# WHDY/SceneDepthEstimation

Hardware: AMD Instinct MI355X
Metric: Mpixel-disparities/sec (H*W*D cost voxels per second, end-to-end per pair) (higher is better)
Workload: dtype f32; 1 GPU; north_star; H=1024, W=1024, D=192, C=64, nlayers=5, pipeline=tower+cv_wta, global_batch=1, parallelism=pairdp1

## Files before the change

include/sde.h:

```cpp
#ifndef SDE_H
#define SDE_H

#include <stddef.h>
#include <stdint.h>

#ifdef __cplusplus
extern "C" {
#endif

#define SDE_ABI_VERSION 4

typedef enum {
    SDE_OK = 0,
    SDE_ERR_ARG = -1,
    SDE_ERR_LAUNCH = -2,
    SDE_ERR_WORKSPACE = -3,
} sde_status;

typedef enum {
    SDE_LAYOUT_DHW = 0,
    SDE_LAYOUT_HWD = 1,
} sde_layout;

typedef enum {
// ... 35 lines not shown
int sde_argmin_merge(const float *mins, const int32_t *args, int nshards, int64_t npix, float *disp,
                     void *stream);


int sde_set_persistent_grid(int cus);

#define SDE_TOWER_FP32 0
#define SDE_TOWER_BF16X6 1
#define SDE_TOWER_F16X3 8
#define SDE_TOWER_WINOGRAD 16
#define SDE_TOWER_MFMA32 32
#define SDE_TOWER_IN_CBLOCK 2
#define SDE_TOWER_OUT_CBLOCK 4
#define SDE_TOWER_IN_SPLIT 64
#define SDE_TOWER_OUT_SPLIT 128

int64_t sde_tower_packed_floats(int nlayers, int nf);

int sde_tower_split_act(void);

int sde_tower_pack_weights(const float *const *hwio, const float *const *biases, int nlayers, int nf,
                           float *packed);

int64_t sde_tower_workspace_bytes(int H, int W, int nlayers, int nf);

int sde_tower_forward(const float *img_pad, int H, int W, const float *packed, int nlayers, int nf,
                      float *feat, void *workspace, int64_t workspace_bytes, int flags, uint16_t *feat_hi,
                      uint16_t *feat_lo, float *feat_norm, void *stream);

int64_t sde_tower_batch_workspace_bytes(int H, int W, int nimg, int nlayers, int nf);
// ... 10 lines not shown

int sde_tower_layer_batch(const float *in, int nimg, int64_t in_stride, int Hin, int Win, const float *packed,
                          int nlayers, int nf, int layer, float *out, int64_t out_stride, int flags,
                          const float *in_absmax, float *out_absmax, int amax_stride, void *stream);

int sde_absmax_f32_batch(const float *x, int nimg, int64_t n, float *absmax, int absmax_stride, void *stream);

int sde_absmax_f32(const float *x, int64_t n, float *absmax, void *stream);

int64_t sde_preprocess_scratch_bytes(int H, int W);
int sde_preprocess_u8(const uint8_t *img, int H, int W, int pad, float *out_pad, void *scratch,
                      void *stream);

int sde_preprocess_u8_batch(const uint8_t *imgs, int nimg, int H, int W, int pad, float *out_pad, void *scratch,
                            void *stream);


int sde_sgm_penalties(const uint8_t *img, int H, int W, double P1, double P2, int64_t threshold,
                      double lambda, float *pen, void *stream);

int sde_sgm_8path(const float *cv, const float *pen, int H, int W, int D, float *S, void *stream);

#define SDE_SGM_ACCUMULATE 1
#define SDE_SGM_ZERO_DU_PENALTIES 2
int sde_sgm_8path_pair(const float *cv_l, const float *pen_l, float *S_l, const float *cv_r, const float *pen_r,
                       float *S_r, int H, int W, int D, int flags, void *stream);

int sde_sgm_8path_wta_pair(const float *cv_l, const float *pen_l, float *S_l, float *disp_l, const float *cv_r,
                           const float *pen_r, float *S_r, float *disp_r, int H, int W, int D, int flags,
                           void *stream);
// ... 36 lines not shown
```

scenedepthestimation_amd/_lib.py:

```python
from __future__ import annotations

import ctypes
import os
import re

import torch

from ._build import INCLUDE, LIB

c_int, c_int64, c_float, c_double, c_void_p = ctypes.c_int, ctypes.c_int64, ctypes.c_float, ctypes.c_double, ctypes.c_void_p
c_char_p = ctypes.c_char_p

SDE_OK = 0
SDE_ABI_VERSION = 4
SDE_LAYOUT_DHW, SDE_LAYOUT_HWD = 0, 1
SDE_WTA_INIT_INF, SDE_WTA_INIT_D0 = 0, 1
SDE_SIDE_LEFT, SDE_SIDE_RIGHT = 1, 2
SDE_TOWER_FP32, SDE_TOWER_BF16X6, SDE_TOWER_F16X3 = 0, 1, 8
SDE_TOWER_IN_CBLOCK, SDE_TOWER_OUT_CBLOCK = 2, 4
SDE_TOWER_WINOGRAD = 16
SDE_TOWER_MFMA32 = 32
SDE_TOWER_IN_SPLIT, SDE_TOWER_OUT_SPLIT = 64, 128
SDE_CV_EXACT, SDE_CV_CERTIFIED = 0, 1
SDE_SGM_ACCUMULATE = 1
SDE_SGM_ZERO_DU_PENALTIES = 2

SIGNATURES = {
    "sde_abi_version": (c_int, []),
    "sde_status_string": (c_char_p, [c_int]),
    "sde_cost_volume": (c_int, [c_void_p, c_void_p, c_int, c_int, c_int, c_int, c_int, c_int, c_float,
                                c_void_p, c_void_p, c_void_p]),
    "sde_wta": (c_int, [c_void_p, c_int, c_int, c_int, c_int, c_int, c_void_p, c_void_p]),
    "sde_cv_wta_workspace_bytes": (c_int64, [c_int, c_int]),
    "sde_cv_wta": (c_int, [c_void_p, c_void_p, c_int, c_int, c_int, c_int, c_int, c_void_p, c_void_p,
                           c_void_p, c_int, c_void_p, c_int64, c_void_p]),
    "sde_feature_split": (c_int, [c_void_p, c_int64, c_int, c_void_p, c_void_p, c_void_p, c_void_p]),
    "sde_cv_wta_split_workspace_bytes": (c_int64, [c_int, c_int]),
# ... 8 lines not shown
    "sde_tower_forward": (c_int, [c_void_p, c_int, c_int, c_void_p, c_int, c_int, c_void_p, c_void_p,
                                  c_int64, c_int, c_void_p, c_void_p, c_void_p, c_void_p]),
    "sde_tower_layer": (c_int, [c_void_p, c_int, c_int, c_void_p, c_int, c_int, c_int, c_void_p, c_int, c_void_p,
                                c_void_p, c_void_p, c_void_p]),
    "sde_tower_batch_workspace_bytes": (c_int64, [c_int, c_int, c_int, c_int, c_int]),
    "sde_tower_forward_batch": (c_int, [c_void_p, c_int, c_int, c_int, c_void_p, c_int, c_int, c_void_p, c_void_p,
                                        c_int64, c_int, c_void_p, c_void_p, c_void_p, c_void_p]),
    "sde_tower_layer_scaled": (c_int, [c_void_p, c_int, c_int, c_void_p, c_int, c_int, c_int, c_void_p, c_int,
                                       c_void_p, c_void_p, c_void_p, c_void_p, c_void_p, c_void_p]),
    "sde_tower_layer_batch": (c_int, [c_void_p, c_int, c_int64, c_int, c_int, c_void_p, c_int, c_int, c_int,
                                      c_void_p, c_int64, c_int, c_void_p, c_void_p, c_int, c_void_p]),
    "sde_absmax_f32": (c_int, [c_void_p, c_int64, c_void_p, c_void_p]),
    "sde_set_persistent_grid": (c_int, [c_int]),
    "sde_absmax_f32_batch": (c_int, [c_void_p, c_int, c_int64, c_void_p, c_int, c_void_p]),
    "sde_preprocess_u8_batch": (c_int, [c_void_p, c_int, c_int, c_int, c_int, c_void_p, c_void_p, c_void_p]),
    "sde_preprocess_u8": (c_int, [c_void_p, c_int, c_int, c_int, c_void_p, c_void_p, c_void_p]),
    "sde_preprocess_scratch_bytes": (c_int64, [c_int, c_int]),
    "sde_sgm_penalties": (c_int, [c_void_p, c_int, c_int, c_double, c_double, c_int64, c_double, c_void_p,
                                  c_void_p]),
    "sde_sgm_8path": (c_int, [c_void_p, c_void_p, c_int, c_int, c_int, c_void_p, c_void_p]),
    "sde_sgm_8path_pair": (c_int, [c_void_p] * 6 + [c_int, c_int, c_int, c_int, c_void_p]),
    "sde_sgm_8path_wta_pair": (c_int, [c_void_p] * 8 + [c_int, c_int, c_int, c_int, c_void_p]),
    "sde_sgm_direction": (c_int, [c_void_p, c_void_p, c_int, c_int, c_int, c_int, c_void_p, c_void_p]),
    "sde_cbca_arms": (c_int, [c_void_p, c_int64, c_int, c_int, c_int, ctypes.c_float, c_void_p, c_void_p]),
    "sde_cbca_workspace_bytes": (ctypes.c_size_t, [c_int, c_int]),
    "sde_cbca": (c_int, [c_void_p] * 4 + [c_int] * 6 + [c_void_p, ctypes.c_size_t, c_void_p]),
    "sde_cbca_pair": (c_int, [c_void_p] * 6 + [c_int] * 5 + [c_void_p, ctypes.c_size_t, c_void_p]),
    "sde_cbca_lr": (c_int, [c_void_p] * 5 + [c_int] * 5 + [c_void_p, ctypes.c_size_t, c_void_p]),
    "sde_cbca_reciprocals": (c_int, [c_void_p, c_int, c_void_p]),
    "sde_lr_check": (c_int, [c_void_p, c_void_p, c_int, c_int, c_void_p, c_void_p, c_void_p]),
# ... 45 lines not shown
```

scenedepthestimation_amd/csrc/cost_volume.hip:

```cpp
#include "sde_common.h"
#include "cv_cert.h"

#include <algorithm>

namespace sde {

constexpr int CV_TX = 64;
constexpr int CV_WAVES = 4;
constexpr int CV_DC = 64;
constexpr int CV_DW = CV_DC / CV_WAVES;
constexpr int CV_ROWS = CV_TX + CV_DC - 1;

enum { OUT_WTA = 0, OUT_DHW = 1, OUT_HWD = 2 };

constexpr int CV_RSTRIDE = 17;

__device__ __forceinline__ float dot64_exact(const float (&own)[64], const float4 *__restrict__ win, int lr)
{
    float acc[8];
    const float4 *row = win + lr * CV_RSTRIDE;
#pragma unroll
    for (int m = 0; m < 8; m++) {
        const float4 a = row[2 * m];
        const float4 b = row[2 * m + 1];
// ... 811 lines not shown
    if (H <= 0 || W <= 0 || d0 < 0 || d1 <= d0 || (!disp && !min_cost && !argmin)) return SDE_ERR_ARG;
    if (!workspace || workspace_bytes < cert_ws_bytes(H, W, false)) return SDE_ERR_WORKSPACE;
    hipStream_t st = as_stream(stream);
    unsigned *counter = reinterpret_cast<unsigned *>(workspace);
    int32_t *list = reinterpret_cast<int32_t *>(reinterpret_cast<char *>(workspace) + 256);
    if (hipMemsetAsync(counter, 0, CERT_COUNTERS * sizeof(unsigned), st) != hipSuccess) return SDE_ERR_LAUNCH;
    cv_wta_cert_kernel<<<cdiv(W, FX_NX) * H, 256, 0, st>>>(
        fl, fr, reinterpret_cast<const uint4 *>(fl_hi), reinterpret_cast<const uint4 *>(fl_lo), fl_norm,
        reinterpret_cast<const uint4 *>(fr_hi), reinterpret_cast<const uint4 *>(fr_lo), fr_norm, H, W, d0, d1,
        min_cost, argmin, disp, counter, list);
    cv_wta_fixup_kernel<<<1024, 256, 0, st>>>(fl, fr, W, d0, d1, counter, list, min_cost, argmin, disp);
    return launch_status();
}

constexpr int ROW_CHUNK = 256;

SDE_EXPORT int sde_cv_wta(const float *fl, const float *fr, int H, int W, int C, int d0, int d1, float *disp,
                          float *min_cost, int32_t *argmin, int mode, void *workspace, int64_t workspace_bytes,
                          void *stream)
{
    if (!fl || !fr || H <= 0 || W <= 0 || C <= 0 || d0 < 0 || d1 <= d0) return SDE_ERR_ARG;
    if (!disp && !min_cost && !argmin) return SDE_ERR_ARG;
    if (mode != SDE_CV_EXACT && mode != SDE_CV_CERTIFIED) return SDE_ERR_ARG;
    hipStream_t st = as_stream(stream);
    auto exact64 = [&] {
        dim3 grid(cdiv(W, CV_TX), H);
        cv64_kernel<SDE_SIDE_LEFT, OUT_WTA><<<grid, 256, 0, st>>>(fl, fr, H, W, d0, d1, 0, -0.0f, nullptr, min_cost,
                                                                   argmin, disp);
    };
    if (C == 64 && mode == SDE_CV_CERTIFIED) {
        if (!workspace || workspace_bytes < sde_cv_wta_workspace_bytes(H, W)) return SDE_ERR_WORKSPACE;
        const int64_t npix = (int64_t)H * W;
        const int K = cdiv(d1 - d0, ROW_CHUNK);
        unsigned *counter = reinterpret_cast<unsigned *>(workspace);
        int32_t *list = reinterpret_cast<int32_t *>(reinterpret_cast<char *>(workspace) + 256);
        if (hipMemsetAsync(counter, 0, CERT_COUNTERS * sizeof(unsigned), st) != hipSuccess) return SDE_ERR_LAUNCH;
        if (row_cert_supported(d0, d1)) {
            launch_row_cert(fl, fr, H, W, d0, d1, min_cost, argmin, disp, counter, list, st);
            cv_wta_fixup_kernel<<<1024, 256, 0, st>>>(fl, fr, W, d0, d1, counter, list, min_cost, argmin, disp);
        } else if (K <= CERT_COUNTERS) {
            float *cmin = reinterpret_cast<float *>(reinterpret_cast<char *>(workspace) + cert_ws_bytes(H, W, false));
            int32_t *carg = reinterpret_cast<int32_t *>(cmin + (size_t)K * npix);
            for (int k = 0; k < K; k++) {
                const int a = d0 + k * ROW_CHUNK, b = std::min(d1, a + ROW_CHUNK);
                float *mk = cmin + (size_t)k * npix;
                int32_t *ak = carg + (size_t)k * npix;
                launch_row_cert(fl, fr, H, W, a, b, mk, ak, nullptr, counter + k, list, st, k > 0 ? mk - npix : nullptr);
                cv_wta_fixup_kernel<<<1024, 256, 0, st>>>(fl, fr, W, a, b, counter + k, list, mk, ak, nullptr);
            }
            argmin_chunks_kernel<<<cdiv(npix, 256), 256, 0, st>>>(cmin, carg, K, npix, disp, min_cost, argmin);
        } else {
            exact64();
        }
    } else if (C == 64) {
        exact64();
// ... 37 lines not shown
```

scenedepthestimation_amd/csrc/cv_row.hip:

```cpp
#include "cv_cert.h"

#include <algorithm>
#include <type_traits>

namespace sde {

constexpr int RW_S = 8;
constexpr float RW_SCALE = (float)(1 << RW_S);
constexpr float RW_K = 1.5e-5f;
constexpr float RW_ABS = 9.3132257e-10f;
constexpr float RW_NMAX = 127.0f;
typedef _Float16 rw_f16x8 __attribute__((ext_vector_type(8)));

__device__ __forceinline__ void rw_split(float x, _Float16 &h, _Float16 &l)
{
    const float xs = x * RW_SCALE;
    h = (_Float16)xs;
    l = (_Float16)(xs - (float)h);
}

__device__ __forceinline__ void rw_split2(float x0, float x1, uint32_t &hi, uint32_t &lo)
{
    typedef _Float16 h2 __attribute__((ext_vector_type(2)));
    const h2 hh = {(_Float16)x0, (_Float16)x1};
    hi = __builtin_bit_cast(uint32_t, hh);
    asm("v_fma_mixlo_f16 %0, %1, 1.0, -%2 op_sel_hi:[0,0,1]" : "=&v"(lo) : "v"(x0), "v"(hi));
    asm("v_fma_mixhi_f16 %0, %1, 1.0, -%2 op_sel:[0,0,1] op_sel_hi:[0,0,1]" : "+v"(lo) : "v"(x1), "v"(hi));
}

constexpr int RW_T = 32;

__device__ __forceinline__ float4 rw_load(const float *__restrict__ frrow, int W, int T, int u)
{
    const int xr = T * RW_T + (u >> 4);
    const bool ok = xr >= 0 && xr < W;
    const float4 v = reinterpret_cast<const float4 *>(frrow)[(size_t)(ok ? xr : 0) * 16 + (u & 15)];
    return ok ? v : make_float4(0.f, 0.f, 0.f, 0.f);
}

template <int CTRL>
__device__ __forceinline__ float rw_dpp(float v)
{
    return __int_as_float(__builtin_amdgcn_update_dpp(0, __float_as_int(v), CTRL, 0xF, 0xF, false));
}

__device__ __forceinline__ bool rw_nonfinite(float x) { return (__float_as_uint(x) & 0x7f800000u) == 0x7f800000u; }

constexpr int R2_NX = 128;
constexpr int R2_NEW = R2_NX / RW_T;
constexpr int R2_LEAD = 2;

__device__ __forceinline__ void r2_load(const float *__restrict__ frrow, int W, int T, int lane, float4 (&v)[8])
{
#pragma unroll
    for (int i = 0; i < 8; i++) v[i] = rw_load(frrow, W, T, lane + 64 * i);
}

__device__ __forceinline__ void r2_store(uint4 *ring, unsigned *tmax, unsigned *tbad, int slot, int lane,
                                         const float4 (&v)[8])
{
    unsigned mx = 0u;
    bool bad = false;
#pragma unroll
    for (int i = 0; i < 8; i++) {
        const int u = lane + 64 * i, px = u >> 4, q = u & 15;
        char *base = reinterpret_cast<char *>(ring + slot * 512 + fx_slot(px, q >> 1)) + 8 * (q & 1);
        const float xs[4] = {v[i].x * RW_SCALE, v[i].y * RW_SCALE, v[i].z * RW_SCALE, v[i].w * RW_SCALE};
        uint32_t hw[2], lw[2];
#pragma unroll
        for (int e = 0; e < 2; e++) rw_split2(xs[2 * e], xs[2 * e + 1], hw[e], lw[e]);
// ... 22 lines not shown
                                                          float *__restrict__ out_min, int32_t *__restrict__ out_arg,
                                                          float *__restrict__ out_disp, unsigned *__restrict__ counter,
                                                          int32_t *__restrict__ list, const float *__restrict__ prev_min)
{
    extern __shared__ __attribute__((aligned(16))) uint4 rsm2[];
    uint4 *ring = rsm2;
    unsigned *tmax = reinterpret_cast<unsigned *>(ring + nt * 512);
    unsigned *tbad = tmax + nt;
    const int y = blockIdx.x;
    const int tid = threadIdx.x, lane = tid & 63;
    const int wave = __builtin_amdgcn_readfirstlane(tid >> 6);
    const int j = lane & 31, h = lane >> 5;
    const float *flrow = fl + (size_t)y * W * 64;
    const float *frrow = fr + (size_t)y * W * 64;
    const size_t rowpix = (size_t)y * W;
    const int nss = (W + R2_NX - 1) / R2_NX;
    auto slot_of = [&](int T) { int r = T % nt; return r < 0 ? r + nt : r; };

    if (wave >= 4) {
        const int sw = wave - 4;
        constexpr int PB = 4;
        float4 nv[8];
#pragma unroll
        for (int b = 0; b < 4 / PB; b++) {
            float4 pv[PB][8];
#pragma unroll
            for (int i = 0; i < PB; i++)
                if (sw + 4 * (PB * b + i) < nw) r2_load(frrow, W, tlo0 + sw + 4 * (PB * b + i), lane, pv[i]);
            if (b == 4 / PB - 1 && nss > 1) r2_load(frrow, W, tlo0 + nw + sw, lane, nv);
#pragma unroll
            for (int i = 0; i < PB; i++)
                if (sw + 4 * (PB * b + i) < nw) r2_store(ring, tmax, tbad, slot_of(tlo0 + sw + 4 * (PB * b + i)), lane, pv[i]);
        }
        __syncthreads();
        for (int k = 0; k < nss; k++) {
            if (k + 1 < nss) {
                const int T = tlo0 + R2_NEW * (k + 1) + nw - R2_NEW + sw;
                r2_store(ring, tmax, tbad, slot_of(T), lane, nv);
                if (k + 2 < nss) r2_load(frrow, W, T + R2_NEW, lane, nv);
            }
            __syncthreads();
        }
        return;
    }

    const int grp = wave & 3;
    float4 lraw[8];
    auto load_left = [&](int kk) {
        const int xx = kk * R2_NX + RW_T * grp + j;
        const float4 *src = reinterpret_cast<const float4 *>(flrow) + (size_t)(xx < W ? xx : 0) * 16 + 2 * h;
#pragma unroll
        for (int s2 = 0; s2 < 4; s2++) { lraw[2 * s2] = src[4 * s2]; lraw[2 * s2 + 1] = src[4 * s2 + 1]; }
    };
    load_left(0);
// ... 243 lines not shown
```

scenedepthestimation_amd/csrc/preprocess.hip:

```cpp
#include "sde_common.h"
#include <algorithm>

namespace sde {

constexpr int NP_PIECE = 8192;

__device__ __forceinline__ float np_val(const uint8_t *img, int64_t i, float mean, bool sq)
{
    const float x = (float)img[i];
    if (!sq) return x;
    const float d = x - mean;
    return d * d;
}

__device__ float np_leaf(const uint8_t *img, int64_t s, int len, float mean, bool sq)
{
    if (len < 8) {
        float res = 0.0f;
        for (int i = 0; i < len; i++) res += np_val(img, s + i, mean, sq);
        return res;
    }
    float r[8];
#pragma unroll
    for (int j = 0; j < 8; j++) r[j] = np_val(img, s + j, mean, sq);
    int i = 8;
    for (; i < len - (len % 8); i += 8) {
#pragma unroll
        for (int j = 0; j < 8; j++) r[j] += np_val(img, s + i + j, mean, sq);
    }
    float res = ((r[0] + r[1]) + (r[2] + r[3])) + ((r[4] + r[5]) + (r[6] + r[7]));
    for (; i < len; i++) res += np_val(img, s + i, mean, sq);
    return res;
}

__device__ __forceinline__ int np_half(int len) { const int n2 = len / 2; return n2 - n2 % 8; }

__device__ __forceinline__ float np_stat(const float *__restrict__ v, int npieces, int64_t n, float *buf, int lane)
{
    float q = 0.0f;
    for (int c0 = 0; c0 < npieces; c0 += 256) {
        const int m = min(256, npieces - c0);
        for (int c = lane; c < m; c += 64) buf[c] = v[c0 + c];
        __builtin_amdgcn_wave_barrier();
        __builtin_amdgcn_fence(__ATOMIC_RELEASE, "wavefront");
        __builtin_amdgcn_wave_barrier();
        if (lane == 0)
            for (int c = 0; c < m; c++) q += buf[c];
        __builtin_amdgcn_wave_barrier();
        __builtin_amdgcn_fence(__ATOMIC_RELEASE, "wavefront");
        __builtin_amdgcn_wave_barrier();
    }
    q = __shfl(q, 0, 64);
    return (float)((double)q / (double)n);
}

template <bool SQ>
__global__ __launch_bounds__(64) void np_piece_kernel(const uint8_t *__restrict__ imgs, int64_t n, int sstride,
                                                      float *__restrict__ scratch)
{
    const uint8_t *img = imgs + blockIdx.y * n;
    float *st = scratch + (size_t)blockIdx.y * sstride;
    const int npieces = gridDim.x;
    __shared__ float sbuf[256];
    float mean = 0.0f;
    if (SQ) {
        mean = np_stat(st + 4, npieces, n, sbuf, threadIdx.x);
        if (blockIdx.x == 0 && threadIdx.x == 0) st[0] = mean;
    }
    const int lane = threadIdx.x;
    const int64_t c0 = (int64_t)blockIdx.x * NP_PIECE;
    const int m = (int)std::min<int64_t>(NP_PIECE, n - c0);
    float sum;
    if (m == NP_PIECE) {
        sum = np_leaf(img, c0 + 128 * lane, 128, mean, SQ);
#pragma unroll
        for (int o = 1; o < 64; o <<= 1) sum += __shfl_xor(sum, o, 64);
    } else {
        __shared__ float leaf[256];
        {
            int ss[16], sl[16], sp = 0, k = 0;
            ss[0] = 0; sl[0] = m;
            while (sp >= 0) {
                const int s0 = ss[sp], len = sl[sp];
                sp--;
                if (len <= 128) {
                    if ((k & 63) == lane) leaf[k] = np_leaf(img, c0 + s0, len, mean, SQ);
                    k++;
                } else {
                    const int n2 = np_half(len);
                    ss[++sp] = s0 + n2; sl[sp] = len - n2;
                    ss[++sp] = s0; sl[sp] = n2;
                }
            }
        }
        __syncthreads();
        sum = 0.0f;
        if (lane == 0) {
            int fl[16], fs[16], sp = 0, k = 0;
            float fv[16], ret = 0.0f;
            fl[0] = m; fs[0] = 0;
            while (sp >= 0) {
// ... 8 lines not shown
                } else if (fs[sp] == 1) {
                    fv[sp] = ret;
                    fs[sp] = 2;
                    const int n2 = np_half(len);
                    ++sp; fl[sp] = len - n2; fs[sp] = 0;
                    continue;
                } else {
                    ret = fv[sp] + ret;
                    sp--;
                }
            }
            sum = ret;
        }
    }
    if (lane == 0) st[4 + (SQ ? npieces : 0) + blockIdx.x] = sum;
}

constexpr int ZN_PER = 8;

__global__ __launch_bounds__(256) void znorm_pad_kernel(const uint8_t *__restrict__ img, int H, int W, int pad,
                                                        float *__restrict__ scratch, int sstride, int npieces,
                                                        float *__restrict__ out)
{
    const int Wp = W + 2 * pad;
    img += (size_t)blockIdx.y * H * W;
    float *st = scratch + (size_t)blockIdx.y * sstride;
    out += (size_t)blockIdx.y * (H + 2 * pad) * Wp;
    __shared__ float sbuf[256];
    __shared__ float sstd;
    if (threadIdx.x < 64) {
        const float v = sqrtf(np_stat(st + 4 + npieces, npieces, (int64_t)H * W, sbuf, threadIdx.x));
        if (threadIdx.x == 0) {
            sstd = v;
            if (blockIdx.x == 0) st[1] = v;
        }
    }
    __syncthreads();
    const float mean = st[0], stdv = sstd;
    const int64_t np_ = (int64_t)(H + 2 * pad) * Wp;
#pragma unroll
    for (int k = 0; k < ZN_PER; k++) {
        const int64_t i = ((int64_t)blockIdx.x * ZN_PER + k) * blockDim.x + threadIdx.x;
        if (i >= np_) break;
        const int ii = (int)i;
        const int y = ii / Wp - pad, x = ii % Wp - pad;
        float v = 0.0f;
        if (y >= 0 && y < H && x >= 0 && x < W) v = ((float)img[(size_t)y * W + x] - mean) / stdv;
        out[i] = v;
    }
}

}

using namespace sde;

SDE_EXPORT int64_t sde_preprocess_scratch_bytes(int H, int W)
{
    if (H <= 0 || W <= 0) return -1;
    const int64_t pieces = ((int64_t)H * W + NP_PIECE - 1) / NP_PIECE;
    return ((4 + 2 * pieces) * 4 + 255) / 256 * 256;
}

SDE_EXPORT int sde_preprocess_u8_batch(const uint8_t *imgs, int nimg, int H, int W, int pad, float *out_pad,
                                       void *scratch, void *stream)
{
    if (!imgs || !out_pad || !scratch || nimg <= 0 || nimg > 65535 || H <= 0 || W <= 0 || pad < 0) return SDE_ERR_ARG;
    const int64_t n = (int64_t)(H + 2 * pad) * (W + 2 * pad);
    if (n >= ((int64_t)1 << 31)) return SDE_ERR_ARG;
    hipStream_t st = as_stream(stream);
    const int64_t npix = (int64_t)H * W;
    const int pieces = (int)((npix + NP_PIECE - 1) / NP_PIECE);
    const int sstride = (int)(sde_preprocess_scratch_bytes(H, W) / 4);
    float *sc = reinterpret_cast<float *>(scratch);
    np_piece_kernel<false><<<dim3(pieces, nimg), 64, 0, st>>>(imgs, npix, sstride, sc);
    np_piece_kernel<true><<<dim3(pieces, nimg), 64, 0, st>>>(imgs, npix, sstride, sc);
    znorm_pad_kernel<<<dim3((unsigned)cdiv(n, 256 * ZN_PER), nimg), 256, 0, st>>>(imgs, H, W, pad, sc, sstride, pieces,
                                                                                  out_pad);
    return launch_status();
}

SDE_EXPORT int sde_preprocess_u8(const uint8_t *img, int H, int W, int pad, float *out_pad, void *scratch,
                                 void *stream)
{
    return sde_preprocess_u8_batch(img, 1, H, W, pad, out_pad, scratch, stream);
}
```

scenedepthestimation_amd/csrc/tower.hip:

```cpp
#include "tower_launch.h"
#include <algorithm>
#include <atomic>

namespace sde {

__global__ __launch_bounds__(256) void absmax_kernel(const float *__restrict__ x, int64_t n, float *__restrict__ amax,
                                                     int amax_stride)
{
    x += blockIdx.y * n;
    amax += blockIdx.y * amax_stride;
    float m = 0.0f;
    const int64_t tid = (int64_t)blockIdx.x * blockDim.x + threadIdx.x, nt = (int64_t)gridDim.x * blockDim.x;
    const int64_t head = std::min<int64_t>(n, (16 - (reinterpret_cast<uintptr_t>(x) & 15)) / 4 & 3);
    if (tid < head) m = fabsf(x[tid]);
    const float4 *x4 = reinterpret_cast<const float4 *>(x + head);
    const int64_t n4 = (n - head) / 4;
    for (int64_t i = tid; i < n4; i += nt) {
        const float4 v = x4[i];
        m = fmaxf(m, fmaxf(fmaxf(fabsf(v.x), fabsf(v.y)), fmaxf(fabsf(v.z), fabsf(v.w))));
    }
    for (int64_t i = head + 4 * n4 + tid; i < n; i += nt) m = fmaxf(m, fabsf(x[i]));
#pragma unroll
    for (int o = 32; o > 0; o >>= 1) m = fmaxf(m, __shfl_xor(m, o, 64));
    __shared__ float red[4];
// ... 98 lines not shown
static bool split_ok(int nlayers, int64_t pix) { return nlayers <= XP_SCALE_WORD && pix < SPLIT_MAX_PIX; }
static bool split_pairing_ok(bool in_sp, bool out_sp, int layer, int nlayers, int Hin, int Win)
{
    if (!in_sp && !out_sp) return true;
    const int sh = layer == 2 ? 4 : 2;
    if ((in_sp && !split_ok(nlayers, (int64_t)Hin * Win)) || (out_sp && !split_ok(nlayers, (int64_t)(Hin - sh) * (Win - sh))))
        return false;
    if ((in_sp && layer == 2) || (out_sp && layer == nlayers)) return false;
    return layer == 2 || layer == nlayers || in_sp == out_sp;
}

SDE_EXPORT int sde_tower_split_act(void) { return SDE_SPLIT_ACT; }

static bool tower_flags_ok(int flags, bool layer_api)
{
    if (flags & (SDE_TOWER_IN_SPLIT | SDE_TOWER_OUT_SPLIT)) {
        if (!layer_api || !(flags & SDE_TOWER_F16X3) || (flags & (SDE_TOWER_WINOGRAD | SDE_TOWER_MFMA32))) return false;
        if ((flags & SDE_TOWER_IN_SPLIT && flags & SDE_TOWER_IN_CBLOCK) ||
            (flags & SDE_TOWER_OUT_SPLIT && flags & SDE_TOWER_OUT_CBLOCK)) return false;
        flags &= ~(SDE_TOWER_IN_SPLIT | SDE_TOWER_OUT_SPLIT);
    }
    if (flags & (SDE_TOWER_WINOGRAD | SDE_TOWER_MFMA32)) {
        if (!(flags & SDE_TOWER_F16X3) || (flags & SDE_TOWER_WINOGRAD && flags & SDE_TOWER_MFMA32)) return false;
        flags &= ~(SDE_TOWER_WINOGRAD | SDE_TOWER_MFMA32);
    }
    const int prec = flags & (SDE_TOWER_BF16X6 | SDE_TOWER_F16X3);
    if (prec == (SDE_TOWER_BF16X6 | SDE_TOWER_F16X3)) return false;
    const int layout = SDE_TOWER_IN_CBLOCK | SDE_TOWER_OUT_CBLOCK;
    if (!layer_api) return (flags & ~(SDE_TOWER_BF16X6 | SDE_TOWER_F16X3)) == 0;
    if (flags & ~(SDE_TOWER_BF16X6 | SDE_TOWER_F16X3 | layout)) return false;
// ... 97 lines not shown
        return launch_status();
    }
    float *buf[2] = {nullptr, nullptr};
    const int64_t h2 = H + 2 * (nlayers - 2), w2 = W + 2 * (nlayers - 2);
    const int64_t act_stride = h2 * w2 * NF;
    if (nlayers > 2) {
        buf[0] = reinterpret_cast<float *>(workspace);
        buf[1] = buf[0] + nimg * act_stride;
    }
    float *amax = reinterpret_cast<float *>(static_cast<char *>(workspace) +
                                            (nlayers > 2 ? 2 * nimg * act_stride * 4 : 0));
    constexpr int AS = (int)(TOWER_AMAX_BYTES / 4);
    const bool f16 = (flags & SDE_TOWER_F16X3) != 0;
    if (f16) {
        if (nlayers > AS) return SDE_ERR_ARG;
        if (hipMemsetAsync(amax, 0, nimg * TOWER_AMAX_BYTES, st) != hipSuccess) return SDE_ERR_LAUNCH;
        const int blocks = (int)std::min<int64_t>(std::max<int64_t>(1, 256 / nimg), cdiv(img_stride, 256 * 16));
        absmax_kernel<<<dim3(blocks, nimg), 256, 0, st>>>(img_pad, img_stride, amax, AS);
    }
    int hin = Hp, win = Wp;
    const bool sp = SDE_SPLIT_ACT && f16 && !(flags & (SDE_TOWER_WINOGRAD | SDE_TOWER_MFMA32)) && nlayers > 2 &&
                    split_ok(nlayers, h2 * w2);
    const bool cbl = !sp && (flags & (SDE_TOWER_BF16X6 | SDE_TOWER_F16X3)) != 0;
    TowerLaunch L{};
    L.ohi = feat_hi, L.olo = feat_lo, L.onrm = feat_norm, L.nimg = nimg, L.bt.amax_stride = AS, L.st = st;
    for (int l = 2; l <= nlayers; l++) {
        const bool first = l == 2, last = l == nlayers;
        L.in = first ? img_pad : buf[(l & 1) ^ 1], L.Hin = hin, L.Win = win, L.out = last ? feat : buf[l & 1];
        L.bt.in_stride = first ? img_stride : act_stride, L.bt.out_stride = last ? feat_stride : act_stride;
        L.in_amax = amax + (l - 2), L.out_amax = amax + (l - 1);
// ... 15 lines not shown
```

scenedepthestimation_amd/ops.py:

```python
from __future__ import annotations

import ctypes

import numpy as np
import torch

from . import _lib
from ._lib import (SDE_LAYOUT_DHW, SDE_LAYOUT_HWD, SDE_SIDE_LEFT, SDE_SIDE_RIGHT, SDE_WTA_INIT_D0,
                   SDE_WTA_INIT_INF, check, lib)

LAYOUTS = {"DHW": SDE_LAYOUT_DHW, "HWD": SDE_LAYOUT_HWD}
RULES = {"inf": SDE_WTA_INIT_INF, "d0": SDE_WTA_INIT_D0}


def _stream() -> int:
    return torch.cuda.current_stream().cuda_stream


def _need(t: torch.Tensor, name: str, dtype=torch.float32, shape=None):
    if not isinstance(t, torch.Tensor):
        raise TypeError(f"{name} must be a torch.Tensor")
    if not t.is_cuda:
        raise ValueError(f"{name} must live on the GPU (got {t.device}); libsde has no CPU path")
    if t.dtype != dtype:
# ... 215 lines not shown
def absmax(x, out):
    check(lib.sde_absmax_f32(_need(x, "absmax input"), x.numel(), _need(out, "absmax word", shape=(1,)), _stream()),
          "sde_absmax_f32")
    return out


def set_persistent_grid(cus: int = 0):
    check(lib.sde_set_persistent_grid(int(cus)), "sde_set_persistent_grid")


def tower_batch_workspace_bytes(H: int, W: int, nimg: int, nlayers: int, nf: int = 64) -> int:
    return int(lib.sde_tower_batch_workspace_bytes(H, W, nimg, nlayers, nf))


def tower_forward_batch(img_pad, packed, nlayers: int, nf: int = 64, out=None, workspace=None,
                        precision: str = "f16x3"):
    N, Hp, Wp = img_pad.shape
    H, W = Hp - 2 * nlayers, Wp - 2 * nlayers
    if H <= 0 or W <= 0:
        raise ValueError("padded image smaller than the tower's receptive field")
    pi = _need(img_pad, "img_pad")
    pw = _need(packed, "packed weights", shape=(tower_packed_floats(nlayers, nf),))
    if out is None:
        out = _empty((N, H, W, nf), torch.float32, img_pad)
    po = _need(out, "features", shape=(N, H, W, nf))
    need = tower_batch_workspace_bytes(H, W, N, nlayers, nf)
    if need > 0 and workspace is None:
        workspace = torch.empty(need, dtype=torch.uint8, device=img_pad.device)
    pws = _need(workspace, "workspace", dtype=torch.uint8) if need > 0 else None
    wsb = workspace.numel() if need > 0 else 0
    check(lib.sde_tower_forward_batch(pi, N, H, W, pw, nlayers, nf, po, pws, wsb, TOWER_PRECISIONS[precision],
                                      None, None, None, _stream()), "sde_tower_forward_batch")
    return out


def absmax_batch(x, out):
    N = x.shape[0]
    _need(x, "absmax input")
    if out.dtype != torch.float32 or not out.is_cuda or out.shape[0] != N or out.stride(1) != 1:
        raise ValueError("absmax words must be a float32 [N, k] device tensor with unit column stride")
    check(lib.sde_absmax_f32_batch(x.data_ptr(), N, x[0].numel(), out.data_ptr(), out.stride(0), _stream()),
          "sde_absmax_f32_batch")
    return out


SCALE_WORD = 32
AMAX_ROW_WORDS = 64
TOWER_SPLIT_ACT = bool(lib.sde_tower_split_act())
# ... 86 lines not shown

def preprocess_u8(img_u8, pad: int, out=None, stats=None):
    H, W = img_u8.shape
    pi = _need(img_u8, "image", dtype=torch.uint8)
    nb = preprocess_scratch_bytes(H, W)
    if out is None:
        out = _empty((H + 2 * pad, W + 2 * pad), torch.float32, img_u8)
    if stats is None:
        stats = _empty((nb,), torch.uint8, img_u8)
    check(lib.sde_preprocess_u8(pi, H, W, pad, _need(out, "out_pad", shape=(H + 2 * pad, W + 2 * pad)),
                                _need(stats, "scratch", dtype=torch.uint8, shape=(nb,)),
                                _stream()), "sde_preprocess_u8")
    return out


def preprocess_u8_batch(imgs_u8, pad: int, out=None, stats=None):
    N, H, W = imgs_u8.shape
    pi = _need(imgs_u8, "images", dtype=torch.uint8)
    nb = N * preprocess_scratch_bytes(H, W)
    if out is None:
        out = _empty((N, H + 2 * pad, W + 2 * pad), torch.float32, imgs_u8)
    if stats is None:
        stats = _empty((nb,), torch.uint8, imgs_u8)
    check(lib.sde_preprocess_u8_batch(pi, N, H, W, pad, _need(out, "out_pad", shape=(N, H + 2 * pad, W + 2 * pad)),
                                      _need(stats, "scratch", dtype=torch.uint8, shape=(nb,)),
                                      _stream()), "sde_preprocess_u8_batch")
    return out


def sgm_penalties(img_u8, P1=2.3, P2=55.9, threshold=30, lamda=4, out=None):
    H, W = img_u8.shape
    pi = _need(img_u8, "image", dtype=torch.uint8)
    if out is None:
        out = _empty((H, W, 16), torch.float32, img_u8)
    check(lib.sde_sgm_penalties(pi, H, W, float(P1), float(P2), int(threshold), float(lamda),
                                _need(out, "penalties", shape=(H, W, 16)), _stream()), "sde_sgm_penalties")
    return out


def sgm_8path(cv_hwd, pen, S=None):
    H, W, D = cv_hwd.shape
# ... 148 lines not shown
```

scenedepthestimation_amd/pipeline.py:

```python
from __future__ import annotations

import numpy as np
import torch

from . import mc_cnn, ops


AMAX_WORDS = ops.AMAX_ROW_WORDS
SPLIT_MAX_PIX = 1 << 24
SGM_PLACEMENT_TRIALS = 16
SGM_PLACEMENT_MIN_VOXELS = 1 << 26
SGM_PLACEMENT_MAX_VOXELS = 1 << 29


def tower_steps(img_pad, packed, nlayers: int, out, ws, precision: str = "f16x3", nf: int = 64, on_launch=None):
    L = nlayers
    N, Hp, Wp = img_pad.shape
    H, W = Hp - 2 * L, Wp - 2 * L
    need = ops.tower_batch_workspace_bytes(H, W, N, L, nf)
    if ws.numel() < need:
        raise ValueError("tower workspace too small")
    h2, w2 = H + 2 * (L - 2), W + 2 * (L - 2)
    sp = ops.TOWER_SPLIT_ACT and precision == "f16x3" and 2 < L <= ops.SCALE_WORD and h2 * w2 < SPLIT_MAX_PIX
    cbl = not sp and precision in ("bf16x6", "f16x3", "f16x3w", "f16x3m32")
    act = h2 * w2 * nf if L > 2 else 0
    wsf = ws[: 2 * N * act * 4 + N * AMAX_WORDS * 4].view(torch.float32)
    bufs = [wsf[: N * act], wsf[N * act: 2 * N * act]]
    words = wsf[2 * N * act:].view(N, AMAX_WORDS)
    f16 = precision in ("f16x3", "f16x3w", "f16x3m32")
    if f16:
        words.zero_()
        ops.absmax_batch(img_pad, words)
    yield 1, words

    def run(layer, fn):
        if on_launch is None:
            fn()
        else:
            on_launch(layer, fn)

    hin, win = H + 2 * L - 4, W + 2 * L - 4
    first = out if L == 2 else bufs[0][: N * hin * win * nf].view(N, hin, win, nf)
    run(2, lambda: ops.tower_layer_batch(img_pad, packed, L, 2, first, nf=nf, precision=precision,
                                         out_cblock=cbl and L > 2, in_absmax=words[:, 0:1] if f16 else None,
                                         out_absmax=words[:, 1:2] if (f16 and L > 2) else None, out_split=sp))
    cur = 0
    for layer in range(3, L + 1):
        yield layer - 1, words
        src = bufs[cur][: N * hin * win * nf].view(N, hin, win, nf)
        o = out if layer == L else bufs[cur ^ 1][: N * (hin - 2) * (win - 2) * nf].view(N, hin - 2, win - 2, nf)
        run(layer, lambda: ops.tower_layer_batch(src, packed, L, layer, o, nf=nf, precision=precision,
                                                 in_cblock=cbl, out_cblock=cbl and layer < L,
                                                 in_absmax=words[:, layer - 2:layer - 1] if f16 else None,
                                                 out_absmax=words[:, layer - 1:layer] if (f16 and layer < L) else None,
                                                 in_split=sp, out_split=sp and layer < L))
        hin, win = hin - 2, win - 2
        cur ^= 1


def run_tower(img_pad, packed, nlayers, out, ws, precision="f16x3", nf=64, combine=None, on_launch=None):
    for _stage, words in tower_steps(img_pad, packed, nlayers, out, ws, precision, nf, on_launch):
        if combine is not None:
            combine(words)
    return out


class StereoMatcher:
    def __init__(self, height: int, width: int, ndisp: int, weights=None, nlayers: int = 5,
                 nf: int = 64, device=None, d_range=None, sgm: bool = False, tower_precision: str = "f16x3",
                 cv_mode: str = "certified", cbca_iters: int = 0, cbca_L1: int = 14, cbca_tau: float = 0.02,
                 emit_split: bool = False, sgm_placement_trials: int = SGM_PLACEMENT_TRIALS):
        self.H, self.W, self.D = int(height), int(width), int(ndisp)
        self.cbca_iters, self.cbca_L1, self.cbca_tau = int(cbca_iters), int(cbca_L1), float(cbca_tau)
        self.nlayers, self.nf = int(nlayers), int(nf)
        self.sgm_placement_trials = int(sgm_placement_trials)
        self.sgm_placement_ms = None
# ... 31 lines not shown
            self._alloc_sgm()

    @property
    def ws(self):
        if self._ws is None:
            nws = ops.tower_batch_workspace_bytes(self.H, self.W, 2, self.nlayers, self.nf)
            self._ws = torch.empty(max(nws, 1), dtype=torch.uint8, device=self.device)
        return self._ws

    def load_images(self, left_u8, right_u8):
        for dst, src in zip(self.img_u8, (left_u8, right_u8)):
            t = src if isinstance(src, torch.Tensor) else torch.from_numpy(np.ascontiguousarray(src, np.uint8))
            dst.copy_(t, non_blocking=False)

    def features(self, on_launch=None):
        ops.preprocess_u8_batch(self.img_u82, self.nlayers, out=self.img_pad2, stats=self.stats2)
        return self.features_from_padded(on_launch)

    def features_from_padded(self, on_launch=None):
        if on_launch is not None and self.split:
            raise ValueError("on_launch needs the layer-by-layer tower, which does not emit split planes "
                             "(emit_split=True): time the one-call tower instead")
        if on_launch is not None:
            run_tower(self.img_pad2, self.packed, self.nlayers, self.feat2, self.ws, self.tower_precision, self.nf,
                      on_launch=on_launch)
            self.split_valid = False
            return self.feat[0], self.feat[1]
        if self.split:
            for i in range(2):
                ops.tower_forward(self.img_pad[i], self.packed, self.nlayers, self.nf, out=self.feat[i],
                                  workspace=self.ws, precision=self.tower_precision, split=self.split[i])
        else:
            ops.tower_forward_batch(self.img_pad2, self.packed, self.nlayers, self.nf, out=self.feat2,
                                    workspace=self.ws, precision=self.tower_precision)
        self.split_valid = self.split is not None
        return self.feat[0], self.feat[1]

    def cost_wta(self, want=("disp",)):
        if self.cv_mode == "certified" and self.split_valid:
            return ops.cv_wta_split(self.feat[0], self.feat[1], self.split[0], self.split[1], self.d0, self.d1,
                                    disp=self.disp if "disp" in want else None,
                                    min_cost=self.min_cost if "min" in want else None,
                                    argmin=self.argmin if "argmin" in want else None, want=(),
                                    workspace=self.cv_ws)
        return ops.cv_wta(self.feat[0], self.feat[1], self.d0, self.d1,
                          disp=self.disp if "disp" in want else None,
                          min_cost=self.min_cost if "min" in want else None,
                          argmin=self.argmin if "argmin" in want else None, want=(),
                          mode=self.cv_mode, workspace=self.cv_ws)
# ... 125 lines not shown
```

Before: 117,900 Mpixel-disparities/s.

## Fuse input absmax into preprocess and use buffer loads in row cost-volume kernel

Preprocessing now tracks the per-image min/max pixel and writes the normalized absmax bound into the tower's amax workspace, so the f16x3 tower can skip its own memset and absmax pass over the padded image. Separately, the row-certified cost-volume kernel swaps guarded global float4 loads for raw buffer loads with a hardware range check, which removes per-load bounds arithmetic. The buffer path is restricted to widths below a limit so the 32-bit offsets stay valid. The added min/max tracking and atomics in preprocessing are a small extra cost.

```diff
diff --git a/include/sde.h b/include/sde.h
--- a/include/sde.h
+++ b/include/sde.h
@@ -73,6 +73,7 @@
 #define SDE_TOWER_OUT_CBLOCK 4
 #define SDE_TOWER_IN_SPLIT 64
 #define SDE_TOWER_OUT_SPLIT 128
+#define SDE_TOWER_BOUND_READY 256
 
 int64_t sde_tower_packed_floats(int nlayers, int nf);
 
@@ -113,6 +114,9 @@
 
 int sde_preprocess_u8_batch(const uint8_t *imgs, int nimg, int H, int W, int pad, float *out_pad, void *scratch,
                             void *stream);
+
+int sde_preprocess_u8_bound_batch(const uint8_t *imgs, int nimg, int H, int W, int pad, float *out_pad, void *scratch,
+                                  float *amax, int amax_stride, int amax_words, void *stream);
 
 
 int sde_sgm_penalties(const uint8_t *img, int H, int W, double P1, double P2, int64_t threshold,
diff --git a/scenedepthestimation_amd/_lib.py b/scenedepthestimation_amd/_lib.py
--- a/scenedepthestimation_amd/_lib.py
+++ b/scenedepthestimation_amd/_lib.py
@@ -21,6 +21,7 @@
 SDE_TOWER_WINOGRAD = 16
 SDE_TOWER_MFMA32 = 32
 SDE_TOWER_IN_SPLIT, SDE_TOWER_OUT_SPLIT = 64, 128
+SDE_TOWER_BOUND_READY = 256
 SDE_CV_EXACT, SDE_CV_CERTIFIED = 0, 1
 SDE_SGM_ACCUMULATE = 1
 SDE_SGM_ZERO_DU_PENALTIES = 2
@@ -59,6 +60,8 @@
     "sde_set_persistent_grid": (c_int, [c_int]),
     "sde_absmax_f32_batch": (c_int, [c_void_p, c_int, c_int64, c_void_p, c_int, c_void_p]),
     "sde_preprocess_u8_batch": (c_int, [c_void_p, c_int, c_int, c_int, c_int, c_void_p, c_void_p, c_void_p]),
+    "sde_preprocess_u8_bound_batch": (c_int, [c_void_p, c_int, c_int, c_int, c_int, c_void_p, c_void_p, c_void_p,
+                                              c_int, c_int, c_void_p]),
     "sde_preprocess_u8": (c_int, [c_void_p, c_int, c_int, c_int, c_void_p, c_void_p, c_void_p]),
     "sde_preprocess_scratch_bytes": (c_int64, [c_int, c_int]),
     "sde_sgm_penalties": (c_int, [c_void_p, c_int, c_int, c_double, c_double, c_int64, c_double, c_void_p,
diff --git a/scenedepthestimation_amd/csrc/cost_volume.hip b/scenedepthestimation_amd/csrc/cost_volume.hip
--- a/scenedepthestimation_amd/csrc/cost_volume.hip
+++ b/scenedepthestimation_amd/csrc/cost_volume.hip
@@ -849,6 +849,7 @@
 }
 
 constexpr int ROW_CHUNK = 256;
+constexpr int ROW_MAX_W = 1 << 23;
 
 SDE_EXPORT int sde_cv_wta(const float *fl, const float *fr, int H, int W, int C, int d0, int d1, float *disp,
                           float *min_cost, int32_t *argmin, int mode, void *workspace, int64_t workspace_bytes,
@@ -870,10 +871,10 @@
         unsigned *counter = reinterpret_cast<unsigned *>(workspace);
         int32_t *list = reinterpret_cast<int32_t *>(reinterpret_cast<char *>(workspace) + 256);
         if (hipMemsetAsync(counter, 0, CERT_COUNTERS * sizeof(unsigned), st) != hipSuccess) return SDE_ERR_LAUNCH;
-        if (row_cert_supported(d0, d1)) {
+        if (W < ROW_MAX_W && row_cert_supported(d0, d1)) {
             launch_row_cert(fl, fr, H, W, d0, d1, min_cost, argmin, disp, counter, list, st);
             cv_wta_fixup_kernel<<<1024, 256, 0, st>>>(fl, fr, W, d0, d1, counter, list, min_cost, argmin, disp);
-        } else if (K <= CERT_COUNTERS) {
+        } else if (W < ROW_MAX_W && K <= CERT_COUNTERS) {
             float *cmin = reinterpret_cast<float *>(reinterpret_cast<char *>(workspace) + cert_ws_bytes(H, W, false));
             int32_t *carg = reinterpret_cast<int32_t *>(cmin + (size_t)K * npix);
             for (int k = 0; k < K; k++) {
diff --git a/scenedepthestimation_amd/csrc/cv_row.hip b/scenedepthestimation_amd/csrc/cv_row.hip
--- a/scenedepthestimation_amd/csrc/cv_row.hip
+++ b/scenedepthestimation_amd/csrc/cv_row.hip
@@ -30,12 +30,18 @@
 
 constexpr int RW_T = 32;
 
-__device__ __forceinline__ float4 rw_load(const float *__restrict__ frrow, int W, int T, int u)
-{
-    const int xr = T * RW_T + (u >> 4);
-    const bool ok = xr >= 0 && xr < W;
-    const float4 v = reinterpret_cast<const float4 *>(frrow)[(size_t)(ok ? xr : 0) * 16 + (u & 15)];
-    return ok ? v : make_float4(0.f, 0.f, 0.f, 0.f);
+__device__ __forceinline__ __amdgpu_buffer_rsrc_t rw_rsrc(const float *row, int W)
+{
+    const uintptr_t b = (uintptr_t)row;
+    const uint32_t lo = __builtin_amdgcn_readfirstlane((uint32_t)b);
+    const uint32_t hi = __builtin_amdgcn_readfirstlane((uint32_t)(b >> 32));
+    return __builtin_amdgcn_make_buffer_rsrc((void *)(((uintptr_t)hi << 32) | lo), 0,
+                                             (int)__builtin_amdgcn_readfirstlane((uint32_t)W * 256u), 0x00020000);
+}
+
+__device__ __forceinline__ float4 rw_load(__amdgpu_buffer_rsrc_t row, uint32_t off)
+{
+    return __builtin_bit_cast(float4, __builtin_amdgcn_raw_buffer_load_b128(row, off, 0, 0));
 }
 
 template <int CTRL>
@@ -50,10 +56,11 @@
 constexpr int R2_NEW = R2_NX / RW_T;
 constexpr int R2_LEAD = 2;
 
-__device__ __forceinline__ void r2_load(const float *__restrict__ frrow, int W, int T, int lane, float4 (&v)[8])
-{
-#pragma unroll
-    for (int i = 0; i < 8; i++) v[i] = rw_load(frrow, W, T, lane + 64 * i);
+__device__ __forceinline__ void r2_load(__amdgpu_buffer_rsrc_t frrow, int T, int lane, float4 (&v)[8])
+{
+    const uint32_t base = (uint32_t)T * (RW_T * 256u) + 16u * (uint32_t)lane;
+#pragma unroll
+    for (int i = 0; i < 8; i++) v[i] = rw_load(frrow, base + 1024u * i);
 }
 
 __device__ __forceinline__ void r2_store(uint4 *ring, unsigned *tmax, unsigned *tbad, int slot, int lane,
@@ -106,6 +113,7 @@
     const float *flrow = fl + (size_t)y * W * 64;
     const float *frrow = fr + (size_t)y * W * 64;
     const size_t rowpix = (size_t)y * W;
+    const __amdgpu_buffer_rsrc_t frbuf = rw_rsrc(frrow, W);
     const int nss = (W + R2_NX - 1) / R2_NX;
     auto slot_of = [&](int T) { int r = T % nt; return r < 0 ? r + nt : r; };
 
@@ -118,8 +126,8 @@
             float4 pv[PB][8];
 #pragma unroll
             for (int i = 0; i < PB; i++)
-                if (sw + 4 * (PB * b + i) < nw) r2_load(frrow, W, tlo0 + sw + 4 * (PB * b + i), lane, pv[i]);
-            if (b == 4 / PB - 1 && nss > 1) r2_load(frrow, W, tlo0 + nw + sw, lane, nv);
+                if (sw + 4 * (PB * b + i) < nw) r2_load(frbuf, tlo0 + sw + 4 * (PB * b + i), lane, pv[i]);
+            if (b == 4 / PB - 1 && nss > 1) r2_load(frbuf, tlo0 + nw + sw, lane, nv);
 #pragma unroll
             for (int i = 0; i < PB; i++)
                 if (sw + 4 * (PB * b + i) < nw) r2_store(ring, tmax, tbad, slot_of(tlo0 + sw + 4 * (PB * b + i)), lane, pv[i]);
@@ -129,7 +137,7 @@
             if (k + 1 < nss) {
                 const int T = tlo0 + R2_NEW * (k + 1) + nw - R2_NEW + sw;
                 r2_store(ring, tmax, tbad, slot_of(T), lane, nv);
-                if (k + 2 < nss) r2_load(frrow, W, T + R2_NEW, lane, nv);
+                if (k + 2 < nss) r2_load(frbuf, T + R2_NEW, lane, nv);
             }
             __syncthreads();
         }
diff --git a/scenedepthestimation_amd/csrc/preprocess.hip b/scenedepthestimation_amd/csrc/preprocess.hip
--- a/scenedepthestimation_amd/csrc/preprocess.hip
+++ b/scenedepthestimation_amd/csrc/preprocess.hip
@@ -5,31 +5,38 @@
 
 constexpr int NP_PIECE = 8192;
 
-__device__ __forceinline__ float np_val(const uint8_t *img, int64_t i, float mean, bool sq)
-{
-    const float x = (float)img[i];
+struct NpRange {
+    unsigned lo = 255u, hi = 0u;
+};
+
+__device__ __forceinline__ float np_val(const uint8_t *img, int64_t i, float mean, bool sq, NpRange &r)
+{
+    const unsigned px = img[i];
+    const float x = (float)px;
     if (!sq) return x;
+    r.lo = min(r.lo, px);
+    r.hi = max(r.hi, px);
     const float d = x - mean;
     return d * d;
 }
 
-__device__ float np_leaf(const uint8_t *img, int64_t s, int len, float mean, bool sq)
+__device__ float np_leaf(const uint8_t *img, int64_t s, int len, float mean, bool sq, NpRange &rg)
 {
     if (len < 8) {
         float res = 0.0f;
-        for (int i = 0; i < len; i++) res += np_val(img, s + i, mean, sq);
+        for (int i = 0; i < len; i++) res += np_val(img, s + i, mean, sq, rg);
         return res;
     }
     float r[8];
 #pragma unroll
-    for (int j = 0; j < 8; j++) r[j] = np_val(img, s + j, mean, sq);
+    for (int j = 0; j < 8; j++) r[j] = np_val(img, s + j, mean, sq, rg);
     int i = 8;
     for (; i < len - (len % 8); i += 8) {
 #pragma unroll
-        for (int j = 0; j < 8; j++) r[j] += np_val(img, s + i + j, mean, sq);
+        for (int j = 0; j < 8; j++) r[j] += np_val(img, s + i + j, mean, sq, rg);
     }
     float res = ((r[0] + r[1]) + (r[2] + r[3])) + ((r[4] + r[5]) + (r[6] + r[7]));
-    for (; i < len; i++) res += np_val(img, s + i, mean, sq);
+    for (; i < len; i++) res += np_val(img, s + i, mean, sq, rg);
     return res;
 }
 
@@ -56,11 +63,18 @@
 
 template <bool SQ>
 __global__ __launch_bounds__(64) void np_piece_kernel(const uint8_t *__restrict__ imgs, int64_t n, int sstride,
-                                                      float *__restrict__ scratch)
+                                                      float *__restrict__ scratch, float *__restrict__ amax,
+                                                      int amax_stride, int amax_words)
 {
     const uint8_t *img = imgs + blockIdx.y * n;
     float *st = scratch + (size_t)blockIdx.y * sstride;
+    unsigned *range = reinterpret_cast<unsigned *>(st + 2);
     const int npieces = gridDim.x;
+    if (!SQ && amax && blockIdx.x == 0) {
+        for (int w = threadIdx.x; w < amax_words; w += 64) amax[(size_t)blockIdx.y * amax_stride + w] = 0.0f;
+        if (threadIdx.x == 0) range[0] = 0u, range[1] = 255u;
+    }
+    NpRange r;
     __shared__ float sbuf[256];
     float mean = 0.0f;
     if (SQ) {
@@ -72,7 +86,7 @@
     const int m = (int)std::min<int64_t>(NP_PIECE, n - c0);
     float sum;
     if (m == NP_PIECE) {
-        sum = np_leaf(img, c0 + 128 * lane, 128, mean, SQ);
+        sum = np_leaf(img, c0 + 128 * lane, 128, mean, SQ, r);
 #pragma unroll
         for (int o = 1; o < 64; o <<= 1) sum += __shfl_xor(sum, o, 64);
     } else {
@@ -84,7 +98,7 @@
                 const int s0 = ss[sp], len = sl[sp];
                 sp--;
                 if (len <= 128) {
-                    if ((k & 63) == lane) leaf[k] = np_leaf(img, c0 + s0, len, mean, SQ);
+                    if ((k & 63) == lane) leaf[k] = np_leaf(img, c0 + s0, len, mean, SQ, r);
                     k++;
                 } else {
                     const int n2 = np_half(len);
@@ -123,13 +137,25 @@
         }
     }
     if (lane == 0) st[4 + (SQ ? npieces : 0) + blockIdx.x] = sum;
+    if (SQ && amax) {
+#pragma unroll
+        for (int o = 1; o < 64; o <<= 1) {
+            r.lo = min(r.lo, (unsigned)__shfl_xor((int)r.lo, o, 64));
+            r.hi = max(r.hi, (unsigned)__shfl_xor((int)r.hi, o, 64));
+        }
+        if (lane == 0) {
+            atomicMax(range, r.hi);
+            atomicMin(range + 1, r.lo);
+        }
+    }
 }
 
 constexpr int ZN_PER = 8;
 
 __global__ __launch_bounds__(256) void znorm_pad_kernel(const uint8_t *__restrict__ img, int H, int W, int pad,
                                                         float *__restrict__ scratch, int sstride, int npieces,
-                                                        float *__restrict__ out)
+                                                        float *__restrict__ out, float *__restrict__ amax,
+                                                        int amax_stride)
 {
     const int Wp = W + 2 * pad;
     img += (size_t)blockIdx.y * H * W;
@@ -141,7 +167,19 @@
         const float v = sqrtf(np_stat(st + 4 + npieces, npieces, (int64_t)H * W, sbuf, threadIdx.x));
         if (threadIdx.x == 0) {
             sstd = v;
-            if (blockIdx.x == 0) st[1] = v;
+            if (blockIdx.x == 0) {
+                st[1] = v;
+                if (amax) {
+                    const unsigned *range = reinterpret_cast<const unsigned *>(st + 2);
+                    const float mean = st[0];
+                    unsigned b = 0u;
+                    for (int e = 0; e < 2; e++) {
+                        const unsigned a = __float_as_uint(((float)range[e] - mean) / v) & 0x7fffffffu;
+                        b = max(b, a > 0x7f800000u ? 0u : a);
+                    }
+                    amax[(size_t)blockIdx.y * amax_stride] = __uint_as_float(b);
+                }
+            }
         }
     }
     __syncthreads();
@@ -170,9 +208,11 @@
     return ((4 + 2 * pieces) * 4 + 255) / 256 * 256;
 }
 
-SDE_EXPORT int sde_preprocess_u8_batch(const uint8_t *imgs, int nimg, int H, int W, int pad, float *out_pad,
-                                       void *scratch, void *stream)
-{
+SDE_EXPORT int sde_preprocess_u8_bound_batch(const uint8_t *imgs, int nimg, int H, int W, int pad, float *out_pad,
+                                             void *scratch, float *amax, int amax_stride, int amax_words,
+                                             void *stream)
+{
+    if (amax && (amax_words < 1 || (nimg > 1 && amax_stride < amax_words))) return SDE_ERR_ARG;
     if (!imgs || !out_pad || !scratch || nimg <= 0 || nimg > 65535 || H <= 0 || W <= 0 || pad < 0) return SDE_ERR_ARG;
     const int64_t n = (int64_t)(H + 2 * pad) * (W + 2 * pad);
     if (n >= ((int64_t)1 << 31)) return SDE_ERR_ARG;
@@ -181,11 +221,17 @@
     const int pieces = (int)((npix + NP_PIECE - 1) / NP_PIECE);
     const int sstride = (int)(sde_preprocess_scratch_bytes(H, W) / 4);
     float *sc = reinterpret_cast<float *>(scratch);
-    np_piece_kernel<false><<<dim3(pieces, nimg), 64, 0, st>>>(imgs, npix, sstride, sc);
-    np_piece_kernel<true><<<dim3(pieces, nimg), 64, 0, st>>>(imgs, npix, sstride, sc);
+    np_piece_kernel<false><<<dim3(pieces, nimg), 64, 0, st>>>(imgs, npix, sstride, sc, amax, amax_stride, amax_words);
+    np_piece_kernel<true><<<dim3(pieces, nimg), 64, 0, st>>>(imgs, npix, sstride, sc, amax, amax_stride, amax_words);
     znorm_pad_kernel<<<dim3((unsigned)cdiv(n, 256 * ZN_PER), nimg), 256, 0, st>>>(imgs, H, W, pad, sc, sstride, pieces,
-                                                                                  out_pad);
+                                                                                  out_pad, amax, amax_stride);
     return launch_status();
+}
+
+SDE_EXPORT int sde_preprocess_u8_batch(const uint8_t *imgs, int nimg, int H, int W, int pad, float *out_pad,
+                                       void *scratch, void *stream)
+{
+    return sde_preprocess_u8_bound_batch(imgs, nimg, H, W, pad, out_pad, scratch, nullptr, 0, 0, stream);
 }
 
 SDE_EXPORT int sde_preprocess_u8(const uint8_t *img, int H, int W, int pad, float *out_pad, void *scratch,
diff --git a/scenedepthestimation_amd/csrc/tower.hip b/scenedepthestimation_amd/csrc/tower.hip
--- a/scenedepthestimation_amd/csrc/tower.hip
+++ b/scenedepthestimation_amd/csrc/tower.hip
@@ -136,6 +136,10 @@
 
 static bool tower_flags_ok(int flags, bool layer_api)
 {
+    if (flags & SDE_TOWER_BOUND_READY) {
+        if (layer_api || !(flags & SDE_TOWER_F16X3)) return false;
+        flags &= ~SDE_TOWER_BOUND_READY;
+    }
     if (flags & (SDE_TOWER_IN_SPLIT | SDE_TOWER_OUT_SPLIT)) {
         if (!layer_api || !(flags & SDE_TOWER_F16X3) || (flags & (SDE_TOWER_WINOGRAD | SDE_TOWER_MFMA32))) return false;
         if ((flags & SDE_TOWER_IN_SPLIT && flags & SDE_TOWER_IN_CBLOCK) ||
@@ -263,6 +267,8 @@
     const bool f16 = (flags & SDE_TOWER_F16X3) != 0;
     if (f16) {
         if (nlayers > AS) return SDE_ERR_ARG;
+    }
+    if (f16 && !(flags & SDE_TOWER_BOUND_READY)) {
         if (hipMemsetAsync(amax, 0, nimg * TOWER_AMAX_BYTES, st) != hipSuccess) return SDE_ERR_LAUNCH;
         const int blocks = (int)std::min<int64_t>(std::max<int64_t>(1, 256 / nimg), cdiv(img_stride, 256 * 16));
         absmax_kernel<<<dim3(blocks, nimg), 256, 0, st>>>(img_pad, img_stride, amax, AS);
diff --git a/scenedepthestimation_amd/ops.py b/scenedepthestimation_amd/ops.py
--- a/scenedepthestimation_amd/ops.py
+++ b/scenedepthestimation_amd/ops.py
@@ -253,7 +253,7 @@
 
 
 def tower_forward_batch(img_pad, packed, nlayers: int, nf: int = 64, out=None, workspace=None,
-                        precision: str = "f16x3"):
+                        precision: str = "f16x3", bound_ready: bool = False):
     N, Hp, Wp = img_pad.shape
     H, W = Hp - 2 * nlayers, Wp - 2 * nlayers
     if H <= 0 or W <= 0:
@@ -268,9 +268,17 @@
         workspace = torch.empty(need, dtype=torch.uint8, device=img_pad.device)
     pws = _need(workspace, "workspace", dtype=torch.uint8) if need > 0 else None
     wsb = workspace.numel() if need > 0 else 0
-    check(lib.sde_tower_forward_batch(pi, N, H, W, pw, nlayers, nf, po, pws, wsb, TOWER_PRECISIONS[precision],
+    flags = TOWER_PRECISIONS[precision] | (_lib.SDE_TOWER_BOUND_READY if bound_ready else 0)
+    check(lib.sde_tower_forward_batch(pi, N, H, W, pw, nlayers, nf, po, pws, wsb, flags,
                                       None, None, None, _stream()), "sde_tower_forward_batch")
     return out
+
+
+def tower_bound_words(workspace, H: int, W: int, nimg: int, nlayers: int, nf: int = 64):
+    h2, w2 = H + 2 * (nlayers - 2), W + 2 * (nlayers - 2)
+    act = h2 * w2 * nf if nlayers > 2 else 0
+    wsf = workspace[2 * nimg * act * 4: 2 * nimg * act * 4 + nimg * AMAX_ROW_WORDS * 4].view(torch.float32)
+    return wsf.view(nimg, AMAX_ROW_WORDS)
 
 
 def absmax_batch(x, out):
@@ -387,7 +395,7 @@
     return out
 
 
-def preprocess_u8_batch(imgs_u8, pad: int, out=None, stats=None):
+def preprocess_u8_batch(imgs_u8, pad: int, out=None, stats=None, bound=None):
     N, H, W = imgs_u8.shape
     pi = _need(imgs_u8, "images", dtype=torch.uint8)
     nb = N * preprocess_scratch_bytes(H, W)
@@ -395,9 +403,16 @@
         out = _empty((N, H + 2 * pad, W + 2 * pad), torch.float32, imgs_u8)
     if stats is None:
         stats = _empty((nb,), torch.uint8, imgs_u8)
-    check(lib.sde_preprocess_u8_batch(pi, N, H, W, pad, _need(out, "out_pad", shape=(N, H + 2 * pad, W + 2 * pad)),
-                                      _need(stats, "scratch", dtype=torch.uint8, shape=(nb,)),
-                                      _stream()), "sde_preprocess_u8_batch")
+    po = _need(out, "out_pad", shape=(N, H + 2 * pad, W + 2 * pad))
+    ps = _need(stats, "scratch", dtype=torch.uint8, shape=(nb,))
+    if bound is None:
+        check(lib.sde_preprocess_u8_batch(pi, N, H, W, pad, po, ps, _stream()), "sde_preprocess_u8_batch")
+        return out
+    if bound.dtype != torch.float32 or not bound.is_cuda or bound.dim() != 2 or bound.shape[0] != N or \
+            bound.shape[1] < 1 or bound.stride(1) != 1 or (N > 1 and bound.stride(0) < bound.shape[1]):
+        raise ValueError("bound words must be a float32 [N, k] device tensor with unit column stride")
+    check(lib.sde_preprocess_u8_bound_batch(pi, N, H, W, pad, po, ps, bound.data_ptr(), bound.stride(0),
+                                            bound.shape[1], _stream()), "sde_preprocess_u8_bound_batch")
     return out
 
 
diff --git a/scenedepthestimation_amd/pipeline.py b/scenedepthestimation_amd/pipeline.py
--- a/scenedepthestimation_amd/pipeline.py
+++ b/scenedepthestimation_amd/pipeline.py
@@ -13,7 +13,8 @@
 SGM_PLACEMENT_MAX_VOXELS = 1 << 29
 
 
-def tower_steps(img_pad, packed, nlayers: int, out, ws, precision: str = "f16x3", nf: int = 64, on_launch=None):
+def tower_steps(img_pad, packed, nlayers: int, out, ws, precision: str = "f16x3", nf: int = 64, on_launch=None,
+                bound_ready: bool = False):
     L = nlayers
     N, Hp, Wp = img_pad.shape
     H, W = Hp - 2 * L, Wp - 2 * L
@@ -28,7 +29,7 @@
     bufs = [wsf[: N * act], wsf[N * act: 2 * N * act]]
     words = wsf[2 * N * act:].view(N, AMAX_WORDS)
     f16 = precision in ("f16x3", "f16x3w", "f16x3m32")
-    if f16:
+    if f16 and not bound_ready:
         words.zero_()
         ops.absmax_batch(img_pad, words)
     yield 1, words
@@ -58,8 +59,9 @@
         cur ^= 1
 
 
-def run_tower(img_pad, packed, nlayers, out, ws, precision="f16x3", nf=64, combine=None, on_launch=None):
-    for _stage, words in tower_steps(img_pad, packed, nlayers, out, ws, precision, nf, on_launch):
+def run_tower(img_pad, packed, nlayers, out, ws, precision="f16x3", nf=64, combine=None, on_launch=None,
+              bound_ready=False):
+    for _stage, words in tower_steps(img_pad, packed, nlayers, out, ws, precision, nf, on_launch, bound_ready):
         if combine is not None:
             combine(words)
     return out
@@ -121,16 +123,19 @@
             dst.copy_(t, non_blocking=False)
 
     def features(self, on_launch=None):
-        ops.preprocess_u8_batch(self.img_u82, self.nlayers, out=self.img_pad2, stats=self.stats2)
-        return self.features_from_padded(on_launch)
-
-    def features_from_padded(self, on_launch=None):
+        bound = None
+        if self.tower_precision.startswith("f16x3") and self.nlayers >= 2 and not self.split:
+            bound = ops.tower_bound_words(self.ws, self.H, self.W, 2, self.nlayers, self.nf)
+        ops.preprocess_u8_batch(self.img_u82, self.nlayers, out=self.img_pad2, stats=self.stats2, bound=bound)
+        return self.features_from_padded(on_launch, bound_ready=bound is not None)
+
+    def features_from_padded(self, on_launch=None, bound_ready=False):
         if on_launch is not None and self.split:
             raise ValueError("on_launch needs the layer-by-layer tower, which does not emit split planes "
                              "(emit_split=True): time the one-call tower instead")
         if on_launch is not None:
             run_tower(self.img_pad2, self.packed, self.nlayers, self.feat2, self.ws, self.tower_precision, self.nf,
-                      on_launch=on_launch)
+                      on_launch=on_launch, bound_ready=bound_ready)
             self.split_valid = False
             return self.feat[0], self.feat[1]
         if self.split:
@@ -139,7 +144,7 @@
                                   workspace=self.ws, precision=self.tower_precision, split=self.split[i])
         else:
             ops.tower_forward_batch(self.img_pad2, self.packed, self.nlayers, self.nf, out=self.feat2,
-                                    workspace=self.ws, precision=self.tower_precision)
+                                    workspace=self.ws, precision=self.tower_precision, bound_ready=bound_ready)
         self.split_valid = self.split is not None
         return self.feat[0], self.feat[1]
 
```

New measurement: 118,100 Mpixel-disparities/s (median of 6 runs). Within noise of the previous version (+0.2%).
